# tarepan/ForwardTacotron

Hardware: AMD Instinct MI355X
Metric: mel-frames/sec at batch=64 LJSpeech shapes (ForwardTacotron.generate, B*T_mel per s) (higher is better)
Workload: dtype fp32; 1 GPU; c3: ForwardTacotron generate, batch=64 per GPU, phoneme lengths U{50..200}; global_batch=64, T_phonemes=200, T_mel=1368, parallelism=dp1

## Files before the change

### forwardtacotron_amd/_lib.py

```python
from __future__ import annotations

import ctypes
import os
from pathlib import Path

import torch

from ._srchash import source_hash

_LIB_PATH = Path(os.environ.get('FTMI_LIB', Path(__file__).resolve().parent / 'libftmi.so'))
_lib = None

c_int, c_int64, c_float, c_void_p = ctypes.c_int32, ctypes.c_int64, ctypes.c_float, ctypes.c_void_p
P = c_void_p
ABI_VERSION = 20
MMA_F32, MMA_BF16X6, MMA_F16X3 = 0, 1, 2


class ConvArgs(ctypes.Structure):
    _fields_ = [
        ('x', P), ('x_stride', c_int64), ('B', c_int), ('T', c_int), ('Cin', c_int),
        ('w', P), ('N', c_int), ('k', c_int), ('pad', c_int),
        ('bias', P), ('relu', c_int), ('bn_scale', P), ('bn_shift', P), ('maxpool', c_int),
        ('residual', P), ('res_stride', c_int64),
        ('y', P), ('y_stride', c_int64), ('yt', P), ('T_out', c_int), ('mma', c_int),
        ('split_k', c_int), ('split_ws', P), ('w_split', P), ('status', P), ('x_split', c_int),
    ]


class WaveRNNArgs(ctypes.Structure):
    _fields_ = [(n, P) for n in ('w_hh1', 'w_hh2', 'w_ih2a', 'w_fc1a', 'w_fc2a', 'w_fc3', 'b_fc3',
                                 'b_hh1', 'b_hh2', 'u1', 'u2', 'v1', 'wm', 'cond', 'mel', 'xin',
                                 'samples', 'logits', 'workspace', 'status')] + [
        ('seed', ctypes.c_uint64)] + [(n, c_int) for n in (
            'bias_row', 'item_rows', 'frames_per_item', 'hop', 'fold_stride', 'batched', 'B', 'L',
            'n_classes', 'mol', 'rnn_dims', 'fc_dims', 'feat_dims', 'aux_dims')]


class TacoArgs(ctypes.Structure):
    _fields_ = [(n, P) for n in (
        'enc', 'enc_proj', 'pre_w1t', 'pre_b1', 'pre_w2t', 'pre_b2', 'gru_wih', 'gru_whh', 'gru_bih',
        'gru_bhh', 'lsa_conv', 'lsa_L', 'lsa_Lb', 'lsa_wt', 'lsa_Wb', 'lsa_v', 'rin_w', 'rin_b',
        'l1_wih', 'l1_whh', 'l1_bih', 'l1_bhh', 'l2_wih', 'l2_whh', 'l2_bih', 'l2_bhh', 'mel_w',
        'pre_gi', 'mel_out', 'attn_out', 'steps_out', 'status', 'workspace', 'stamps')] + [
        ('stop_threshold', c_float)] + [(n, c_int) for n in (
            'B', 'T', 'r', 'steps', 'decoder_dims', 'lstm_dims', 'n_mels', 'prenet_dims')]


class NnlsArgs(ctypes.Structure):
    _fields_ = [('mel', P)] + [(n, c_int) for n in ('B', 'F', 'n_mels', 'n_bins', 'denorm')] + [
        ('blocks', P)] + [(n, c_int) for n in ('n_blocks', 'groups', 'm', 'max_frames', 'maxiter', 'dbg_stop')] + [
        (n, P) for n in ('rowvals', 'rowptr', 'rowlo', 'bin_rows', 'bin_w', 'pinv', 'workspace', 'S',
                         'active')]


SIGNATURES = {
    'ftmi_abi_version': (c_int, []),
    'ftmi_build_id': (ctypes.c_char_p, []),
    'ftmi_strerror': (ctypes.c_char_p, [c_int]),
    'ftmi_set_resident_cu_limit': (c_int, [c_int]),
    'ftmi_embedding': (c_int, [P, c_int64, P, c_int64, c_int64, P, P, P]),
    'ftmi_conv1d': (c_int, [ctypes.POINTER(ConvArgs), P]),
    'ftmi_conv_bank': (c_int, [P, c_int64, c_int, c_int, c_int, P, P, c_int, c_int, P, P, P, c_int64,
                               c_int, P, P]),
    'ftmi_conv_bank_split': (c_int, [P, c_int64, c_int, c_int, c_int, P, P, c_int, c_int, P, P, P,
                                     c_int64, c_int, P, c_int, P, c_int, P]),
    'ftmi_conv_bank_halves_ws_floats': (c_int64, [c_int, c_int, c_int, c_int]),
    'ftmi_conv_bank_halves_image_bytes': (c_int64, [c_int, c_int, c_int]),
    'ftmi_conv_bank_halves_image': (c_int, [P, c_int, c_int, c_int, P, P]),
    'ftmi_highway': (c_int, [P, c_int64, c_int64, c_int, P, P, P, P, P, c_int64, c_int, P, P]),
    'ftmi_highway_split': (c_int, [P, c_int64, c_int64, c_int, P, P, P, P, P, c_int64, c_int, P,
                                   c_int, P, P]),
    'ftmi_highway_stack': (c_int, [P, c_int64, c_int64, c_int, c_int, P, c_int, P, P, P, P, P,
                                   c_int, P, c_int64, P, c_int64, P, P]),
    'ftmi_highway_stack_spread_ws_bytes': (c_int64, [c_int64]),
    'ftmi_highway_stack_spread_blocks': (c_int, [c_int64]),
    'ftmi_highway_stack_spread': (c_int, [P, c_int64, c_int64, c_int, c_int, P, c_int, P, P, P, P,
                                          P, c_int, P, c_int64, P, c_int64, P, P, P]),
    'ftmi_split_weights_bytes': (c_int64, [c_int64, c_int64]),
    'ftmi_split_weights': (c_int, [P, c_int64, c_int64, P, P]),
    'ftmi_split_weights_f16_bytes': (c_int64, [c_int64, c_int64]),
    'ftmi_split_rows': (c_int, [P, c_int64, c_int64, c_int, P, c_int64, P, P]),
    'ftmi_split_weights_f16': (c_int, [P, c_int64, c_int64, P, P]),
    'ftmi_split_weights_f16_frag': (c_int, [P, c_int64, c_int64, P, P]),
    'ftmi_panel_proj': (c_int, [P, c_int64, c_int64, c_int, P, c_int, P, P, c_int64, P, P,
                                c_float, P, c_int64, P, P]),
    'ftmi_rnn_workspace_bytes': (c_int64, [c_int, c_int, c_int]),
    'ftmi_rnn_error_offset': (c_int64, [c_int]),
    'ftmi_rnn_blocks': (c_int, [c_int, c_int, c_int, c_int]),
    'ftmi_set_rnn_spin_limit': (ctypes.c_uint32, [ctypes.c_uint32]),
    'ftmi_rnn_bidir': (c_int, [c_int, c_int, c_int, c_int, P, c_int64, c_int, P, P, P, P, P,
                               c_float, P, c_int64, c_int, P, P, P]),
    'ftmi_duration_counts': (c_int, [P, c_int, c_int, c_int, c_float, P, P, P, P]),
    'ftmi_duration_trunc_sum': (c_int, [P, c_int, c_int, P, P]),
    'ftmi_duration_counts_global': (c_int, [P, c_int, c_int, P, c_float, P, P, P, P]),
    'ftmi_lr_index': (c_int, [P, c_int, c_int, c_int, P, P]),
    'ftmi_length_regulate': (c_int, [P, c_int64, c_int, c_int, c_int, P, c_int, P, c_int64, P]),
    'ftmi_series_proj_add': (c_int, [P, c_int64, c_int, c_int, c_int, P, P, P, c_float, P, P, P,
                                     c_float, P]),
    'ftmi_rowdot': (c_int, [P, c_int64, c_int64, c_int, P, P, c_float, P, P]),
    'ftmi_embedding_posenc': (c_int, [P, c_int, c_int, P, c_int64, c_int, P, P, P, P, P]),
    'ftmi_lr_posenc': (c_int, [P, c_int64, c_int, c_int, c_int, P, c_int, P, P, P, c_int64, P]),
    'ftmi_layernorm': (c_int, [P, c_int64, c_int64, c_int, P, P, c_float, P, c_int64, P]),
    'ftmi_attention': (c_int, [P, c_int64, c_int, c_int, c_int, c_int, c_int, c_int, c_int, P,
                               c_float, P, c_int64, c_int, P, P, c_int64, P]),
    'ftmi_panel_proj_qkv': (c_int, [P, c_int64, c_int, c_int, c_int, P, c_int, P, c_int, P,
                                    c_int64, P, c_int64, P, P]),
    'ftmi_attention_kv': (c_int, [P, c_int64, c_int, c_int, c_int, c_int, P, c_float, P, c_int64,
                                  P, P, c_int64, P]),
    'ftmi_attention_workspace_bytes': (c_int64, [c_int, c_int, c_int, c_int]),
    'ftmi_stft': (c_int, [P, c_int64, c_int, c_int64, P, c_int, c_int, P, P, c_int, P, P, P]),
    'ftmi_mel_spectrogram': (c_int, [P, c_int64, c_int, c_int64, P, c_int, c_int, P, P, c_int, P,
                                     P, P, P, c_int, c_int, P, P]),
    'ftmi_griffinlim_stft': (c_int, [P, c_int64, c_int, c_int64, P, c_int, c_int, P, P, c_int, P,
                                     P, P, c_float, c_int, P, P]),
    'ftmi_spec_mul': (c_int, [P, P, c_int64, P, P]),
    'ftmi_unit_phases': (c_int, [P, c_int, c_int, c_int, P, P]),
    'ftmi_istft_workspace_bytes': (c_int64, [c_int, c_int, c_int]),
    'ftmi_istft': (c_int, [P, c_int, c_int, P, c_int, c_int, P, P, P, P, P, c_int64, c_int64, P]),
    'ftmi_griffinlim_iter': (c_int, [P, P, P, P, c_int, c_int, P, c_int, c_int, P, P, P, c_float,
                                     c_int, P]),
    'ftmi_istft_fused': (c_int, [P, c_int, c_int, P, c_int, c_int, P, P, P, P, c_int64, c_int64, P]),
    'ftmi_wr_stretch_conv': (c_int, [P, c_int64, c_int, c_int, c_int, c_int, P, P, c_int64, c_int,
                                     c_int, P]),
    'ftmi_wavernn_workspace_bytes': (c_int64, []),
    'ftmi_wavernn': (c_int, [ctypes.POINTER(WaveRNNArgs), P]),
    'ftmi_set_wavernn_spin_limit': (ctypes.c_uint32, [ctypes.c_uint32]),
    'ftmi_wr_unfold': (c_int, [P, c_int, c_int, c_int, c_int, c_int, c_int, c_int, c_int, c_int, P, P]),
    'ftmi_tacotron_decoder_workspace_bytes': (c_int64, [c_int, c_int]),
    'ftmi_tacotron_decoder': (c_int, [ctypes.POINTER(TacoArgs), P]),
    'ftmi_align_workspace_bytes': (c_int64, [c_int, c_int, c_int]),
    'ftmi_align_dijkstra': (c_int, [P, c_int64, c_int64, c_int, c_int, c_int, P, P, P, P, P, P]),
    'ftmi_align_count': (c_int, [P, c_int64, c_int64, c_int, c_int, c_int, P, P, P, P]),
    'ftmi_attention_score': (c_int, [P, c_int64, c_int64, c_int, c_int, c_int, P, c_int, P, P, P]),
    'ftmi_phoneme_features': (c_int, [P, c_int64, c_int64, c_int, c_int, c_int, P, P, c_int64, c_int,
                                      P, P, c_int64, c_int, P, c_float, P, P, P, P]),
    'ftmi_nonzero_moments': (c_int, [P, c_int64, P, P]),
    'ftmi_normalize_nonzero': (c_int, [P, c_int64, c_float, c_float, P]),
    'ftmi_mel_nnls': (c_int, [P, c_int, c_int, P, c_int, c_int, c_int, c_int, P, P, P, P, P, P,
                              c_float, c_int, P, P]),
    'ftmi_nnls_lbfgsb_workspace_bytes': (c_int64, [c_int, c_int, c_int, c_int, c_int]),
    'ftmi_nnls_lbfgsb_start': (c_int, [ctypes.POINTER(NnlsArgs), P]),
    'ftmi_nnls_lbfgsb_cycles': (c_int, [ctypes.POINTER(NnlsArgs), c_int, P]),
    'ftmi_nnls_lbfgsb_finish': (c_int, [ctypes.POINTER(NnlsArgs), P, P, P, P]),
}


class FtmiError(RuntimeError):
    pass


def lib_path() -> Path:
# ... 32 lines not shown
```

### forwardtacotron_amd/common_layers.py

```python
from __future__ import annotations

import math
from typing import List, Optional

import torch
import torch.nn as nn

from . import ops



def _uniform_(t: torch.Tensor, bound: float) -> None:
    with torch.no_grad():
        t.uniform_(-bound, bound)


class Conv1dParams(nn.Module):

    def __init__(self, cin: int, cout: int, k: int, bias: bool) -> None:
        super().__init__()
        self.in_channels, self.out_channels, self.kernel_size = cin, cout, k
        self.weight = nn.Parameter(torch.empty(cout, cin, k))
        self.bias = nn.Parameter(torch.empty(cout)) if bias else None
        b = 1.0 / math.sqrt(cin * k)
# ... 146 lines not shown

class BiRNN(Packed):

    def __init__(self, fin: int, hidden: int, cell: str) -> None:
        super().__init__()
        self.cell = 0 if cell == 'gru' else 1
        self.input_size, self.hidden = fin, hidden
        self.spread = False
        gh = (3 if self.cell == 0 else 4) * hidden
        b = 1.0 / math.sqrt(hidden)
        for sfx in ('', '_reverse'):
            for name, shape in (('weight_ih_l0', (gh, fin)), ('weight_hh_l0', (gh, hidden)),
                                ('bias_ih_l0', (gh,)), ('bias_hh_l0', (gh,))):
                prm = nn.Parameter(torch.empty(*shape))
                _uniform_(prm, b)
                self.register_parameter(name + sfx, prm)

    def _pack(self):
        w_ih = torch.cat([self.weight_ih_l0, self.weight_ih_l0_reverse], 0).detach().contiguous()
        b_ih = torch.cat([self.bias_ih_l0, self.bias_ih_l0_reverse], 0).detach().contiguous()
        b_hh = torch.cat([self.bias_hh_l0, self.bias_hh_l0_reverse], 0).detach().contiguous()
        w_hh = torch.stack([self.weight_hh_l0, self.weight_hh_l0_reverse], 0).detach().contiguous()
        if self.cell == 1:
            return w_ih, (b_ih + b_hh).contiguous(), None, w_hh, presplit(w_ih)
        return w_ih, b_ih, b_hh, w_hh, presplit(w_ih)

    def forward_cl(self, x: torch.Tensor, T: Optional[int] = None, index=None, lengths=None,
                   pad_value: float = 0.0) -> torch.Tensor:
        return self.recur(self.project(x), T=T, index=index, lengths=lengths,
                          pad_value=pad_value)

    def project(self, x: torch.Tensor) -> torch.Tensor:
        w_ih, b_in, _, _, w3 = self.packed_weights()
        xp, _ = ops.conv1d(x, w_ih, 1, 0, bias=b_in, w_split=w3)
        return xp

    def recur(self, xp: torch.Tensor, T: Optional[int] = None, index=None, lengths=None,
              pad_value: float = 0.0) -> torch.Tensor:
        _, b_in, b_hh, w_hh, _ = self.packed_weights()
        return ops.rnn_bidir(self.cell, xp, self.hidden, w_hh, b_hh, T=T, index=index,
                             xp_zero=b_in if index is not None else None, lengths=lengths,
                             pad_value=pad_value, spread=self.spread)

    def forward(self, x: torch.Tensor):
        return self.forward_cl(x.contiguous()), None


class CBHG(Packed):

    def __init__(self, K: int, in_channels: int, channels: int, proj_channels: List[int],
                 num_highways: int, dropout: float = 0.5) -> None:
        super().__init__()
        self.dropout = dropout
        self.K = K
        self.channels = channels
        self.bank_kernels = list(range(1, K + 1))
        self.conv1d_bank = nn.ModuleList(
            [BatchNormConv(in_channels, channels, k) for k in self.bank_kernels])
        self.conv_project1 = BatchNormConv(K * channels, proj_channels[0], 3)
        self.conv_project2 = BatchNormConv(proj_channels[0], proj_channels[1], 3, relu=False)
        self.pre_highway = LinearParams(proj_channels[-1], channels, bias=False)
        self.highways = nn.ModuleList([HighwayNetwork(channels) for _ in range(num_highways)])
        self.rnn = GRUParamsModule(channels, channels)

    def _pack(self):
        ws = [pack_conv(c.conv.weight) for c in self.conv1d_bank]
        bank_w = torch.cat([w.reshape(-1) for w in ws]).contiguous()
        folds = [c.bnorm.folded() for c in self.conv1d_bank]
        scale = torch.cat([f[0] for f in folds]).contiguous()
        shift = torch.cat([f[1] for f in folds]).contiguous()
        w_pre = self.pre_highway.weight.detach().contiguous()
        bank3 = ops.split_bank_weights(bank_w, self.K, ws[0].size(1), self.channels)
        img = ops.bank_halves_image(bank3, self.K, ws[0].size(1), self.channels)
        return bank_w, scale, shift, w_pre, bank3, presplit(w_pre), img

    def forward_cl(self, x: torch.Tensor) -> torch.Tensor:
        bank_w, scale, shift, w_pre, bank3, pre3, img = self.packed_weights()
        pooled = ops.bank_pools(x, self.K, self.channels, w_split=bank3)
        split = pooled and ops.SPLIT_ROWS
        xin = pooled and ops.SPLIT_BANK_IN
        bank = ops.conv_bank(ops.split_rows(x) if xin else x, bank_w, self.K, self.channels,
                             scale, shift, w_split=bank3, pool=pooled, split_out=split,
                             x_split=xin, w_image=img)
        y = self.conv_project1.forward_cl(bank, maxpool=not pooled, x_split=split)
        del bank
        y = self.conv_project2.forward_cl(y, residual=x)
        xp = self._highway_stack(y)
        if xp is not None:
            return self.rnn.recur(xp)
        h, _ = ops.conv1d(y, w_pre, 1, 0, w_split=pre3)
        h2 = torch.empty_like(h)
        for hw in self.highways:
            hw.forward_cl(h, out=h2)
            h, h2 = h2, h
        return self.rnn.forward_cl(h)

    def _stack_pack(self):
        key = self._pack_key()
        cache = self.__dict__.get('_ftmi_stack')
        if cache is None or cache[0] != key:
            with torch.no_grad():
                w_pre = self.packed_weights()[3]
                hw = [m.packed_weights() for m in self.highways]
                w_ih, b_in = self.rnn.packed_weights()[:2]
                f16 = ops.split_weights_f16
                cache = (key, (f16(w_pre, frag=True), [f16(p[0], frag=True) for p in hw],
                               [p[1] for p in hw], [p[2] for p in hw], f16(w_ih, frag=True),
                               b_in, w_ih.size(0)))
            self.__dict__['_ftmi_stack'] = cache
        return cache[1]

    def spread_blocks(self, M: int) -> int:
        Cp = self.channels
        if not ops.highway_stack_ok(M, Cp, self.channels, len(self.highways), 6 * self.channels,
                                    (self.packed_weights()[5],)):
            return 0
        return ops.hs_spread_blocks(M, 6 * self.channels)

    def _highway_stack(self, y: torch.Tensor) -> Optional[torch.Tensor]:
        M, Cp = y.size(0) * y.size(1), y.size(2)
        n_out = 6 * self.channels
        if not ops.highway_stack_ok(M, Cp, self.channels, len(self.highways), n_out,
                                    (self.packed_weights()[5],)):
            return None
        pre_f, hw_f, b1s, b2s, ih_f, b_in, n_out = self._stack_pack()
        xp, _ = ops.highway_stack(y, pre_f, self.channels, hw_f, b1s, b2s, ih_f, b_in, n_out,
                                  spread=getattr(self, 'allow_spread', True))
        return xp

    def forward(self, x: torch.Tensor) -> torch.Tensor:
        return self.forward_cl(x.transpose(1, 2).contiguous())


class GRUParamsModule(BiRNN):

    def __init__(self, fin: int, hidden: int) -> None:
        super().__init__(fin, hidden, 'gru')


class LSTMParamsModule(BiRNN):

    def __init__(self, fin: int, hidden: int) -> None:
        super().__init__(fin, hidden, 'lstm')
```

### forwardtacotron_amd/forward_tacotron.py

```python
from __future__ import annotations

import os
from pathlib import Path
from typing import Any, Callable, Dict, Union

import numpy as np
import torch
import torch.nn as nn

from . import ops
from .common_layers import (CBHG, BatchNormConv, BiRNN, Conv1dParams, LengthRegulator,
                            LinearParams, Packed, pack_conv)
from .text.symbols import phonemes


def _identity(t: torch.Tensor) -> torch.Tensor:
    return t


def graph_safe(fn: Callable[[torch.Tensor], torch.Tensor]) -> Callable[[torch.Tensor], torch.Tensor]:
    fn._ftmi_graph_safe = True
    return fn


# ... 180 lines not shown
        pitch = batch['pitch'].unsqueeze(1)
        energy = batch['energy'].unsqueeze(1)
        with torch.no_grad():
            dur_hat = self.dur_pred.forward_bt(x)
            pitch_hat = self.pitch_pred.forward_bt(x).unsqueeze(1)
            energy_hat = self.energy_pred.forward_bt(x).unsqueeze(1)
            enc = self._encode(x, pitch, energy)
            dur_c = dur.float().contiguous()
            offsets, totals, _ = ops.duration_counts(dur_c, apply_fill=False)
            if dur_c.data_ptr() != dur.data_ptr():
                dur.copy_(dur_c)
            lens = mel_lens.to(torch.int64)
            T_pack = int(lens.max().item())
            if T_pack > int(totals.max().item()):
                raise RuntimeError('mel_len exceeds the length-regulated sequence length')
            index = ops.lr_index(offsets, T_pack)
            x_mel, x_post = self._decode(enc, index, lengths=lens.to(x.device))
            x_post = self._pad(x_post, mel.size(2))
            x_mel = self._pad(x_mel, mel.size(2))
        return {'mel': x_mel, 'mel_post': x_post,
                'dur': dur_hat, 'pitch': pitch_hat, 'energy': energy_hat}

    def _side_streams(self, device, B: int, T: int = 0):
        cache = self.__dict__.setdefault('_ftmi_streams', {})
        if device not in cache:
            prio = int(os.environ.get('FTMI_PRENET_PRIORITY', '-1'))
            cache[device] = [torch.cuda.Stream(device=device), torch.cuda.Stream(device=device),
                             torch.cuda.Stream(device=device, priority=prio)]
        fits = self.__dict__.setdefault('_ftmi_concurrent', {})
        key = (device, B, T, ops.RNN_MMA, bool(ops._FORCED), os.environ.get('FTMI_HS_SPREAD', '1'))
        if key not in fits:
            preds = (self.dur_pred.rnn, self.pitch_pred.rnn, self.energy_pred.rnn)
            need = sum(ops.rnn_blocks(r.cell, B, r.hidden) for r in preds)
            pre = ops.rnn_blocks(self.prenet.rnn.cell, B, self.prenet.rnn.hidden)
            spread = self.prenet.spread_blocks(B * T)
            cus = ops._num_cus()
            use_spread = spread > 0 and need + max(pre, spread) <= cus
            fits[key] = (0 < need + pre <= cus and pre > 0, use_spread)
        concurrent, use_spread = fits[key]
        self.prenet.allow_spread = use_spread
        if not concurrent:
            main = torch.cuda.current_stream(device)
            return [main, main, main]
        return cache[device]

    def _weights_key(self):
        refs = self.__dict__.get('_ftmi_wrefs')
        if refs is None or any(d.get(n) is not t for d, n, t in refs):
            refs = [(d, n, t) for m in self.modules() for d in (m._parameters, m._buffers)
                    for n, t in d.items() if t is not None]
            self.__dict__['_ftmi_wrefs'] = refs
        return tuple((t.data_ptr(), t._version) for _, _, t in refs)

    def _phoneme_graph(self, x, alpha, pitch_fn, energy_fn):
        cache = self.__dict__.setdefault('_ftmi_graphs', {})
        seen = self.__dict__.setdefault('_ftmi_graph_seen', {})
        split = not (_graphable(pitch_fn) and _graphable(energy_fn))
        key = ((x.device, tuple(x.shape), float(alpha), 'split', ops.MMA, ops.RNN_MMA) if split else
               (x.device, tuple(x.shape), float(alpha), pitch_fn, energy_fn, ops.MMA, ops.RNN_MMA))
        cap_p, cap_e = (None, None) if split else (pitch_fn, energy_fn)
        ent = cache.pop(key, None)
        fresh = False
        if ent is None:
            n = seen.get(key, 0)
            if n < 0:
                return None
            if len(seen) >= 64 * GRAPH_CACHE:
                seen.clear()
            seen[key] = n + 1
            if n == 0:
                return None
            wkey = self._weights_key()
            sx = x.clone()
            try:
                self._phoneme_phase(sx, alpha, cap_p, cap_e, capture=True)
                torch.cuda.synchronize(x.device)
                g = torch.cuda.CUDAGraph()
                with torch.cuda.graph(g):
                    outs = self._phoneme_phase(sx, alpha, cap_p, cap_e, capture=True)
            except Exception:
                torch.cuda.synchronize(x.device)
                seen[key] = -1
                return None
            packs = [m.__dict__.get('_ftmi_pack') for m in self.modules()]
            ent = {'g': g, 'sx': sx, 'outs': outs, 'wkey': wkey, 'packs': packs,
                   'done': torch.cuda.Event()}
            ent['done'].record(torch.cuda.current_stream(x.device))
            fresh = True
            while len(cache) >= GRAPH_CACHE:
                cache.pop(next(iter(cache)))
        cache[key] = ent
        main = torch.cuda.current_stream(x.device)
        main.wait_event(ent['done'])
        ent['sx'].copy_(x)
        ent['g'].replay()
        if not fresh and self._weights_key() != ent['wkey']:
            main.synchronize()
            cache.clear()
            return None
        dur_hat, pitch_hat, energy_hat, enc, offsets, tmax, xp = ent['outs']
        t_host = torch.empty((), dtype=tmax.dtype, pin_memory=True)
        t_host.copy_(tmax, non_blocking=True)
        t_ready = torch.cuda.Event()
        t_ready.record(main)
        dur_hat, pitch_hat, energy_hat = dur_hat.clone(), pitch_hat.clone(), energy_hat.clone()
        if split:
            pitch_hat, energy_hat = pitch_fn(pitch_hat), energy_fn(energy_hat)
            wp, bp, we, be = self._folded_series_weights()
            ops.series_proj_add(xp, pitch_hat, wp, bp, self.pitch_strength, energy_hat, we,
                                be, self.energy_strength)
        t_ready.synchronize()
        return (dur_hat, pitch_hat, energy_hat, enc, offsets, int(t_host), xp), ent

    def _phoneme_phase(self, x, alpha, pitch_fn, energy_fn, batch=None, capture=False):
        main = torch.cuda.current_stream(x.device)
        s_pitch, s_energy, s_prenet = self._side_streams(x.device, x.size(0), x.size(1))
        for s in (s_pitch, s_energy, s_prenet):
            s.wait_stream(main)
        with torch.cuda.stream(s_prenet):
            enc = self.prenet.forward_cl(ops.embedding(x, self.embedding.weight.detach()))
            xp = self.lstm.project(enc)
        dur_hat = self.dur_pred.forward_bt(x, alpha=alpha)
        t_host = t_ready = None
        tmax = None
        if batch is None and capture:
            offsets, totals, _ = ops.duration_counts(dur_hat, apply_fill=True)
            tmax = totals.max()
        elif batch is None:
            offsets, totals, _ = ops.duration_counts(dur_hat, apply_fill=True)
            t_host = torch.empty((), dtype=totals.dtype, pin_memory=True)
            t_host.copy_(totals.max(), non_blocking=True)
            t_ready = torch.cuda.Event()
            t_ready.record(main)
        with torch.cuda.stream(s_pitch):
            pitch_hat = self.pitch_pred.forward_bt(x).unsqueeze(1)
            if pitch_fn is not None:
                pitch_hat = pitch_fn(pitch_hat)
        with torch.cuda.stream(s_energy):
            energy_hat = self.energy_pred.forward_bt(x).unsqueeze(1)
            if energy_fn is not None:
                energy_hat = energy_fn(energy_hat)
        if pitch_fn is not None and energy_fn is not None:
            with torch.cuda.stream(s_prenet):
                for s, t in ((s_pitch, pitch_hat), (s_energy, energy_hat)):
                    s_prenet.wait_stream(s)
                    if not capture:
                        t.record_stream(s_prenet)
                wp, bp, we, be = self._folded_series_weights()
                ops.series_proj_add(xp, pitch_hat, wp, bp, self.pitch_strength, energy_hat, we,
                                    be, self.energy_strength)
        if batch is not None:
            offsets, totals = batch.duration_counts(dur_hat)
            T_mel = batch.t_mel(totals)
        index = None
        if not capture:
            if t_ready is not None:
                t_ready.synchronize()
                T_mel = int(t_host)
            index = ops.lr_index(offsets, T_mel)
        for s, ts in ((s_pitch, (pitch_hat,)), (s_energy, (energy_hat,)),
                      (s_prenet, (enc, xp))):
            main.wait_stream(s)
            if not capture:
                for t in ts:
                    t.record_stream(main)
        if capture:
            return dur_hat, pitch_hat, energy_hat, enc, offsets, tmax, xp
        return dur_hat, pitch_hat, energy_hat, enc, (offsets, index), T_mel, xp

    def generate(self,
                 x: torch.Tensor,
                 alpha=1.0,
                 pitch_function: Callable[[torch.Tensor], torch.Tensor] = _identity,
                 energy_function: Callable[[torch.Tensor], torch.Tensor] = _identity,
                 batch=None) -> Dict[str, torch.Tensor]:
        if self.training:
            self.eval()
        self._check_device(x)

        graph = GRAPH and batch is None and x.numel() <= GRAPH_MAX_TOKENS

        def run():
            with torch.no_grad():
                phase = ent = None
                if graph and not ops.forced_exact():
                    r = self._phoneme_graph(x, alpha, pitch_function, energy_function)
                    if r is not None:
                        phase, ent = r
                if phase is None:
                    phase = self._phoneme_phase(x, alpha, pitch_function, energy_function, batch)
                dur_hat, pitch_hat, energy_hat, enc, offsets, T_mel, xp = phase
                out = self._generate_mel(x, dur_hat, pitch_hat, energy_hat, enc=enc,
                                         lr=(offsets, T_mel), xp=xp)
                if ent is not None:
                    ent['done'].record(torch.cuda.current_stream(x.device))
                return out
        return ops.run_checked(run, x.device, reduce=None if batch is None else batch.status)

    def __prepare_scriptable__(self):
        from .jit import ScriptedForwardTacotron
        return ScriptedForwardTacotron(self)

    def generate_jit(self, x: torch.Tensor, alpha: float = 1.0, beta: float = 1.0) -> Dict[str, torch.Tensor]:
        self._check_device(x)

        def run():
            with torch.no_grad():
                dur_hat, pitch_hat, energy_hat, enc, offsets, T_mel, xp = self._phoneme_phase(
                    x, alpha, lambda p: p * beta, lambda e: e)
                return self._generate_mel(x, dur_hat, pitch_hat, energy_hat, enc=enc,
                                          lr=(offsets, T_mel), xp=xp)
        return ops.run_checked(run, x.device)

    def get_step(self) -> int:
        return self.step.data.item()

    def _generate_mel(self, x, dur_hat, pitch_hat, energy_hat, enc=None, lr=None, xp=None):
        if enc is None:
            enc = self.prenet.forward_cl(ops.embedding(x, self.embedding.weight.detach()))
        if xp is None:
            wp, bp, we, be = self._series_proj_weights()
            ops.series_proj_add(enc, pitch_hat, wp, bp, self.pitch_strength, energy_hat, we, be,
                                self.energy_strength)
        index = None
        if lr is None:
            offsets, totals, _ = ops.duration_counts(dur_hat, apply_fill=False)
            T_mel = int(totals.max().item())
        else:
            offsets, T_mel = lr
            if isinstance(offsets, tuple):
                offsets, index = offsets
        if index is None:
            index = ops.lr_index(offsets, T_mel)
        mel, mel_post = self._decode(enc, index, xp=xp)
        return {'mel': mel, 'mel_post': mel_post, 'dur': dur_hat,
                'pitch': pitch_hat, 'energy': energy_hat}

    def _pad(self, x: torch.Tensor, max_len: int) -> torch.Tensor:
        x = x[:, :, :max_len]
        if x.size(2) < max_len:
            pad = torch.full((x.size(0), x.size(1), max_len - x.size(2)), self.padding_value,
                             device=x.device, dtype=x.dtype)
            x = torch.cat([x, pad], 2)
        return x

    @classmethod
    def from_config(cls, config: Dict[str, Any]) -> 'ForwardTacotron':
        model_config = config['forward_tacotron']['model']
        model_config['num_chars'] = len(phonemes)
        model_config['n_mels'] = config['dsp']['num_mels']
        return ForwardTacotron(**model_config)

    @classmethod
    def from_checkpoint(cls, path: Union[Path, str]) -> 'ForwardTacotron':
        checkpoint = torch.load(path, map_location=torch.device('cpu'), weights_only=True)
        model = ForwardTacotron.from_config(checkpoint['config'])
        model.load_state_dict(checkpoint['model'])
        return model
```

### forwardtacotron_amd/ops.py

```python
from __future__ import annotations

import contextlib
import ctypes
import os
from typing import Optional, Tuple

import numpy as np
import torch

from . import _lib
from ._lib import ConvArgs
from .probe import launch

_f32 = torch.float32

MMA = int(os.environ.get('FTMI_MMA', '2'))
RNN_MMA = int(os.environ.get('FTMI_RNN_MMA', '2'))

STATUS_F16_RANGE, STATUS_WHH_RANGE, STATUS_RNN_TIMEOUT = 1, 2, 4
_STATUS = {}
_FORCED = []


def status_word(device) -> torch.Tensor:
# ... 284 lines not shown
                      Cout: int) -> Optional[torch.Tensor]:
    if (w_split is None or w_split.dtype != torch.uint8 or not w_split.is_cuda
            or os.environ.get('FTMI_BANK_IMAGE', '1') == '0'):
        return None
    lib = _lib.load()
    n = int(lib.ftmi_conv_bank_halves_image_bytes(Cin, K, Cout))
    if n <= 0:
        return None
    img = torch.empty(n, device=w_split.device, dtype=torch.uint8)
    launch('ftmi_conv_bank_halves_image', f'bank_halves_image[K={K},Cin={Cin},Cout={Cout}]', 0,
           2.0 * n, w_split.data_ptr(), Cin, K, Cout, img.data_ptr(), _stream())
    return img


def conv_bank(x: torch.Tensor, w: torch.Tensor, K: int, Cout: int, scale: torch.Tensor,
              shift: torch.Tensor, mma: Optional[int] = None,
              w_split: Optional[torch.Tensor] = None, pool: bool = False,
              split_out: bool = False, x_split: bool = False,
              w_image: Optional[torch.Tensor] = None) -> torch.Tensor:
    if split_out and not pool:
        raise ValueError('split_out needs pool')
    _dev(x, w, scale, shift, w_split)
    B, T, Cin, xs = _rows(x)
    y = torch.empty(B, T, K * Cout, device=x.device, dtype=_f32)
    M = B * T
    flops = 2.0 * M * Cout * Cin * K * (K + 1) / 2
    mma, wsp = _gemm_mma(mma, w_split)
    sk, part, last = 0, None, 0
    if not pool and not x_split and _bank_halves(mma, B, T, Cin, K, Cout):
        n = int(_lib.load().ftmi_conv_bank_halves_ws_floats(B, T, K, Cout)) - BANK_COUNTERS
        sk, part, last = 2, _bank_workspace(n, x.device), BANK_HALVES
        if w_image is not None:
            _dev(w_image)
            wsp, last = w_image.data_ptr(), BANK_HALVES | BANK_IMAGE
    elif not pool and _skinny(mma, T, T, Cin, K, M) and _skinny_split(Cin) > 1:
        sk = _skinny_split(Cin)
        part = torch.empty(sk * M * K * Cout, device=x.device, dtype=_f32)
    launch('ftmi_conv_bank_split', f'conv_bank[M={M},K={K},Cin={Cin},mma={mma}'
           f'{",pool" if pool else ""}{",split" if split_out else ""}{",xsplit" if x_split else ""}'
           ']',
           flops, 4.0 * (M * Cin + Cout * Cin * K * (K + 1) / 2 + M * K * Cout),
           x.data_ptr(), xs, B, T, Cin, w.data_ptr(), wsp, K, Cout,
           scale.data_ptr(), shift.data_ptr(), y.data_ptr(), y.stride(-2), mma,
           status_word(x.device).data_ptr(), sk, _ptr(part),
           int(pool) | (2 * int(split_out)) | (4 * int(x_split)) | last, _stream())
    return y


BANK_COUNTERS = 4096
BANK_HALVES, BANK_IMAGE = 16, 32


def _bank_halves(mma: int, B: int, T: int, Cin: int, K: int, Cout: int) -> bool:
    return (os.environ.get('FTMI_BANK_HALVES', '1') != '0' and mma == 2 and 0 < B * T <= 128
            and Cin % 64 == 0 and Cin <= 256 and K % 2 == 0 and Cout % 16 == 0
            and (K // 2) * (Cout // 16) % 8 == 0 and (K // 2) * (Cout // 16) <= 512 and K <= 16)
_BANK_WS = {}


def _bank_workspace(n_part: int, device) -> torch.Tensor:
    stream = torch.cuda.current_stream(device)
    key = (torch.device(device), stream.cuda_stream)
    t = _BANK_WS.get(key)
    if t is None or t.numel() < BANK_COUNTERS + n_part:
        if t is not None:
            _BANK_OLD.append(t)
        t = _BANK_WS[key] = torch.zeros(BANK_COUNTERS + n_part, device=device, dtype=_f32)
    return t


_BANK_OLD = []


def split_rows(x: torch.Tensor) -> torch.Tensor:
    _dev(x)
    B, T, C, xs = _rows(x)
    y = torch.empty(B, T, C, device=x.device, dtype=_f32)
    launch('ftmi_split_rows', f'split_rows[M={B * T},C={C}]', 0.0, 8.0 * B * T * C,
           x.data_ptr(), xs, B * T, C, y.data_ptr(), y.stride(1),
           status_word(x.device).data_ptr(), _stream())
    return y


def highway(x: torch.Tensor, w12: torch.Tensor, b1: torch.Tensor, b2: torch.Tensor,
            out: Optional[torch.Tensor] = None, mma: Optional[int] = None,
            w_split: Optional[torch.Tensor] = None) -> torch.Tensor:
    _dev(x, w12, b1, b2, out, w_split)
    B, T, C, xs = _rows(x)
    y = out if out is not None else torch.empty(B, T, C, device=x.device, dtype=_f32)
    M = B * T
    mma, wsp = _gemm_mma(mma, w_split)
    sk, part = 0, None
    if (mma == 2 and wsp is not None and os.environ.get('FTMI_GEMM_SKINNY', '1') != '0'
            and C % 16 == 0 and 0 < M <= SKINNY_MMAX_NARROW):
        sk = _skinny_split(C)
        part = torch.empty(sk * M * 2 * C, device=x.device, dtype=_f32)
    launch('ftmi_highway_split', f'highway[M={M},C={C},mma={mma}]', 2.0 * M * 2 * C * C,
           4.0 * (2 * M * C + 2 * C * C),
           x.data_ptr(), xs, M, C, w12.data_ptr(), wsp, b1.data_ptr(),
           b2.data_ptr(), y.data_ptr(), y.stride(1), mma, status_word(x.device).data_ptr(),
           sk, _ptr(part), _stream())
    return y


HS_C, HS_NPASS, HS_MAXL = 256, 512, 8
HS_MIN_ROWS = int(os.environ.get('FTMI_HS_MIN', 64))


def highway_stack_ok(M: int, Cp: int, C: int, L: int, n_out: int, splits) -> bool:
    if os.environ.get('FTMI_HS', '1') == '0' or (_FORCED and _FORCED[-1][0] != 2):
        return False
    if not _FORCED and MMA != 2:
        return False
    return (C == HS_C and 0 < Cp <= C and Cp % 4 == 0 and L <= HS_MAXL
            and n_out % HS_NPASS == 0 and M >= max(HS_MIN_ROWS, 1)
            and all(w is not None and w.dtype == torch.uint8 for w in splits))


def highway_stack(x: torch.Tensor, pre_split: torch.Tensor, C: int, hw_splits, b1s, b2s,
                  out_split: Optional[torch.Tensor], b_out: Optional[torch.Tensor], n_out: int,
                  want_h: bool = False, spread: bool = True):
    _dev(x, pre_split, out_split, b_out, *hw_splits, *b1s, *b2s)
    B, T, Cp, xs = _rows(x)
    M = B * T
    L = len(hw_splits)
    y = torch.empty(B, T, n_out, device=x.device, dtype=_f32) if out_split is not None else None
    h = torch.empty(B, T, C, device=x.device, dtype=_f32) if want_h else None
    arr = ctypes.c_void_p * max(L, 1)
    w_arr = arr(*[w.data_ptr() for w in hw_splits])
    b1_arr = arr(*[b.data_ptr() for b in b1s])
    b2_arr = arr(*[b.data_ptr() for b in b2s])
    flops = 2.0 * M * C * (Cp + L * 2 * C + n_out)
    nbytes = 4.0 * M * (Cp + n_out + (C if want_h else 0))
    args = (x.data_ptr(), xs, M, Cp, C, pre_split.data_ptr(), L, ctypes.addressof(w_arr),
            ctypes.addressof(b1_arr), ctypes.addressof(b2_arr), _ptr(out_split), _ptr(b_out),
            n_out if out_split is not None else 0, _ptr(y), y.stride(1) if y is not None else 0,
            _ptr(h), h.stride(1) if h is not None else 0, status_word(x.device).data_ptr())
    if spread and hs_spread_blocks(M, n_out if out_split is not None else 0) > 0:
        ws = _spread_workspace(int(_lib.load().ftmi_highway_stack_spread_ws_bytes(M)), x.device)
        launch('ftmi_highway_stack_spread', f'highway_stack_spread[M={M},Cp={Cp},L={L},N={n_out}]',
               flops, nbytes, *args, ws.data_ptr(), _stream())
    else:
        launch('ftmi_highway_stack', f'highway_stack[M={M},Cp={Cp},L={L},N={n_out}]', flops,
               nbytes, *args, _stream())
    return y, h


def hs_spread_blocks(M: int, n_out: int = 0) -> int:
    if os.environ.get('FTMI_HS_SPREAD', '1') == '0' or n_out > 1536:
        return 0
    n = int(_lib.load().ftmi_highway_stack_spread_blocks(M))
    return n if 0 < n <= _num_cus() else 0


_SPREAD_WS = {}


def _spread_workspace(nbytes: int, device) -> torch.Tensor:
    stream = torch.cuda.current_stream(device)
    key = (torch.device(device), stream.cuda_stream)
    t = _SPREAD_WS.get(key)
    if t is None or t.numel() < nbytes:
        if t is not None:
            _BANK_OLD.append(t)
        t = _SPREAD_WS[key] = torch.zeros(max(nbytes, 16), device=device, dtype=torch.uint8)
    return t
# ... 487 lines not shown
```

### include/ftmi.h

```cpp
#ifndef FTMI_H
#define FTMI_H

#include <stdint.h>

#ifdef __cplusplus
extern "C" {
#endif

typedef void *ftmi_stream_t;

enum {
  FTMI_OK = 0,
  FTMI_E_ARG = 1001,
  FTMI_E_SHAPE = 1002,
  FTMI_E_UNSUPPORTED = 1003,
  FTMI_E_ALIGN = 1004
};

enum { FTMI_MMA_F32 = 0, FTMI_MMA_BF16X6 = 1, FTMI_MMA_F16X3 = 2 };

enum { FTMI_STATUS_F16_RANGE = 1, FTMI_STATUS_WHH_RANGE = 2, FTMI_STATUS_RNN_TIMEOUT = 4 };

enum { FTMI_BANK_POOL = 1,
       FTMI_BANK_Y_SPLIT = 2,
       FTMI_BANK_X_SPLIT = 4,
       FTMI_BANK_HALVES = 16,
       FTMI_BANK_IMAGE = 32    };
enum { FTMI_BANK_COUNTERS = 4096 };

int ftmi_abi_version(void);
const char *ftmi_build_id(void);
const char *ftmi_strerror(int code);
int32_t ftmi_set_resident_cu_limit(int32_t cus);

int ftmi_embedding(const int64_t *ids, int64_t n, const float *table, int64_t num_rows,
                   int64_t dim, float *out, int32_t *err, ftmi_stream_t stream);

typedef struct ftmi_conv_args {
  const float *x;
  int64_t x_stride;
  int32_t B, T, Cin;
  const float *w;
  int32_t N, k, pad;
  const float *bias;
  int32_t relu;
  const float *bn_scale;
  const float *bn_shift;
  int32_t maxpool;
  const float *residual;
  int64_t res_stride;
  float *y;
  int64_t y_stride;
  float *yt;
  int32_t T_out;
  int32_t mma;
  int32_t split_k;
  float *split_ws;
  const void *w_split;
  uint32_t *status;
  int32_t x_split;
} ftmi_conv_args;


int64_t ftmi_split_weights_bytes(int64_t N, int64_t K);
int ftmi_split_weights(const float *w, int64_t N, int64_t K, void *out, ftmi_stream_t stream);

int64_t ftmi_split_weights_f16_bytes(int64_t N, int64_t K);
int ftmi_split_weights_f16(const float *w, int64_t N, int64_t K, void *out,
                           ftmi_stream_t stream);

int ftmi_conv1d(const ftmi_conv_args *args, ftmi_stream_t stream);

int ftmi_conv_bank(const float *x, int64_t x_stride, int32_t B, int32_t T, int32_t Cin,
                   const float *w, const void *w_split, int32_t K, int32_t Cout,
                   const float *bn_scale,
                   const float *bn_shift, float *y, int64_t y_stride, int32_t mma,
                   uint32_t *status, ftmi_stream_t stream);

int64_t ftmi_conv_bank_halves_ws_floats(int32_t B, int32_t T, int32_t K, int32_t Cout);
int64_t ftmi_conv_bank_halves_image_bytes(int32_t Cin, int32_t K, int32_t Cout);
int ftmi_conv_bank_halves_image(const void *w_split, int32_t Cin, int32_t K, int32_t Cout,
                                void *image, ftmi_stream_t stream);
int ftmi_conv_bank_split(const float *x, int64_t x_stride, int32_t B, int32_t T, int32_t Cin,
                         const float *w, const void *w_split, int32_t K, int32_t Cout,
                         const float *bn_scale, const float *bn_shift, float *y,
                         int64_t y_stride, int32_t mma, uint32_t *status, int32_t split_k,
                         float *split_ws, int32_t pool_out, ftmi_stream_t stream);

int ftmi_highway(const float *x, int64_t x_stride, int64_t M, int32_t C, const float *w12,
                 const void *w12_split, const float *b1, const float *b2, float *y,
                 int64_t y_stride, int32_t mma, uint32_t *status, ftmi_stream_t stream);

int ftmi_highway_split(const float *x, int64_t x_stride, int64_t M, int32_t C,
                       const float *w12, const void *w12_split, const float *b1,
                       const float *b2, float *y, int64_t y_stride, int32_t mma,
                       uint32_t *status, int32_t split_k, float *split_ws,
                       ftmi_stream_t stream);

int ftmi_split_weights_f16_frag(const float *w, int64_t N, int64_t K, void *out,
                                ftmi_stream_t stream);

int ftmi_split_rows(const float *x, int64_t x_stride, int64_t rows, int32_t C, float *y,
                    int64_t y_stride, uint32_t *status, ftmi_stream_t stream);

int ftmi_highway_stack(const float *x, int64_t x_stride, int64_t M, int32_t Cp, int32_t C,
                       const void *w_pre_split, int32_t L, const void *const *w_hw_split,
                       const float *const *b1, const float *const *b2,
                       const void *w_out_split, const float *b_out, int32_t n_out, float *y,
                       int64_t y_stride, float *h, int64_t h_stride, uint32_t *status,
                       ftmi_stream_t stream);

int64_t ftmi_highway_stack_spread_ws_bytes(int64_t M);
int32_t ftmi_highway_stack_spread_blocks(int64_t M);
int ftmi_highway_stack_spread(const float *x, int64_t x_stride, int64_t M, int32_t Cp,
                              int32_t C, const void *w_pre_split, int32_t L,
                              const void *const *w_hw_split, const float *const *b1,
                              const float *const *b2, const void *w_out_split,
                              const float *b_out, int32_t n_out, float *y, int64_t y_stride,
                              float *h, int64_t h_stride, uint32_t *status, void *ws,
                              ftmi_stream_t stream);

enum { FTMI_RNN_SPREAD = 0x100 };
int64_t ftmi_rnn_workspace_bytes(int32_t B, int32_t H, int32_t cell);
int64_t ftmi_rnn_error_offset(int32_t B);
int32_t ftmi_rnn_blocks(int32_t cell, int32_t B, int32_t H, int32_t mma);
uint32_t ftmi_set_rnn_spin_limit(uint32_t limit);
int ftmi_rnn_bidir(int32_t cell, int32_t B, int32_t T, int32_t H, const float *xp,
                   int64_t xp_stride, int32_t T_src, const int32_t *index,
                   const float *xp_zero, const float *w_hh, const float *b_hh,
                   const int32_t *lengths, float pad_value, float *y, int64_t y_stride,
                   int32_t mma, uint32_t *status, void *sync, ftmi_stream_t stream);

int ftmi_duration_counts(float *dur, int32_t B, int32_t T, int32_t apply_fill,
                         float fill_value, int32_t *offsets, int32_t *totals,
                         int32_t *fill_flag, ftmi_stream_t stream);

int ftmi_duration_trunc_sum(const float *dur, int32_t B, int32_t T, int64_t *out,
                            ftmi_stream_t stream);
int ftmi_duration_counts_global(float *dur, int32_t B, int32_t T, const int64_t *global_sum,
                                float fill_value, int32_t *offsets, int32_t *totals,
                                int32_t *fill_flag, ftmi_stream_t stream);

int ftmi_lr_index(const int32_t *offsets, int32_t B, int32_t T, int32_t T_mel,
                  int32_t *index, ftmi_stream_t stream);

int ftmi_length_regulate(const float *x, int64_t x_stride, int32_t B, int32_t T, int32_t C,
                         const int32_t *index, int32_t T_mel, float *y, int64_t y_stride,
                         ftmi_stream_t stream);

int ftmi_series_proj_add(float *x, int64_t x_stride, int32_t B, int32_t T, int32_t C,
                         const float *pitch, const float *wp, const float *bp,
                         float pitch_strength, const float *energy, const float *we,
                         const float *be, float energy_strength, ftmi_stream_t stream);

int ftmi_rowdot(const float *x, int64_t x_stride, int64_t M, int32_t C, const float *w,
                const float *bias, float alpha, float *out, ftmi_stream_t stream);


int ftmi_stft(const float *y, int64_t y_stride, int32_t B, int64_t L, const int32_t *lengths,
              int32_t n_fft, int32_t hop, const double *window, const void *twiddle, int32_t F,
              const int32_t *frames, void *X, ftmi_stream_t stream);

int ftmi_mel_spectrogram(const float *y, int64_t y_stride, int32_t B, int64_t L,
                         const int32_t *lengths, int32_t n_fft, int32_t hop, const double *window,
                         const void *twiddle, int32_t F, const int32_t *frames, const float *basis,
                         const int32_t *mel_lo, const int32_t *mel_hi, int32_t n_mels,
                         int32_t log_norm, float *mel, ftmi_stream_t stream);

int ftmi_griffinlim_stft(const float *y, int64_t y_stride, int32_t B, int64_t L,
                         const int32_t *lengths, int32_t n_fft, int32_t hop, const double *window,
                         const void *twiddle, int32_t F, const int32_t *frames, const float *S,
// ... 162 lines not shown
```

Baseline: 10.99 million mel-frames/s.

## Fold embedding into CBHG conv bank via precomputed per-token tap table

Because the prenet CBHG conv bank's input is an embedding lookup, each bank convolution output becomes a sum of precomputed rows, one per (token id, tap), from a table built as embedding times conv weight. A new kernel gathers and sums these rows, then applies ReLU, batchnorm, maxpool and the optional f16 split output, replacing the conv-bank GEMM. The table is cached per weight version and registered with the graph pack list. It trades matmul compute for table memory and gather bandwidth, which grows with vocab times taps times Cout.

```diff
diff --git a/forwardtacotron_amd/_lib.py b/forwardtacotron_amd/_lib.py
--- a/forwardtacotron_amd/_lib.py
+++ b/forwardtacotron_amd/_lib.py
@@ -68,6 +68,8 @@
     'ftmi_conv_bank_halves_ws_floats': (c_int64, [c_int, c_int, c_int, c_int]),
     'ftmi_conv_bank_halves_image_bytes': (c_int64, [c_int, c_int, c_int]),
     'ftmi_conv_bank_halves_image': (c_int, [P, c_int, c_int, c_int, P, P]),
+    'ftmi_embed_bank': (c_int, [P, c_int, c_int, P, c_int, c_int, c_int, c_int, P, P, P, c_int64,
+                                c_int, P, P]),
     'ftmi_highway': (c_int, [P, c_int64, c_int64, c_int, P, P, P, P, P, c_int64, c_int, P, P]),
     'ftmi_highway_split': (c_int, [P, c_int64, c_int64, c_int, P, P, P, P, P, c_int64, c_int, P,
                                    c_int, P, P]),
diff --git a/forwardtacotron_amd/common_layers.py b/forwardtacotron_amd/common_layers.py
--- a/forwardtacotron_amd/common_layers.py
+++ b/forwardtacotron_amd/common_layers.py
@@ -252,6 +252,35 @@
         bank = ops.conv_bank(ops.split_rows(x) if xin else x, bank_w, self.K, self.channels,
                              scale, shift, w_split=bank3, pool=pooled, split_out=split,
                              x_split=xin, w_image=img)
+        return self._after_bank(bank, x, pooled, split)
+
+    def embed_bank_table(self, embedding_weight: torch.Tensor) -> torch.Tensor:
+        key = (self._pack_key(), embedding_weight.data_ptr(), embedding_weight._version,
+               embedding_weight.device)
+        cache = self.__dict__.get('_ftmi_embed_table')
+        if cache is None or cache[0] != key:
+            with torch.no_grad():
+                cache = (key, ops.embed_bank_table(
+                    embedding_weight, [c.conv.weight for c in self.conv1d_bank]))
+            self.__dict__['_ftmi_embed_table'] = cache
+        return cache[1]
+
+    def forward_ids(self, x_ids: torch.Tensor, embedding_weight: torch.Tensor) -> torch.Tensor:
+        w = embedding_weight.detach()
+        h = ops.embedding(x_ids, w)
+        if (x_ids.numel() < ops.EMBED_BANK_MIN_ROWS
+                or w.size(1) != self.conv1d_bank[0].conv.in_channels
+                or not ops.embed_bank_ok(w.size(0), 1, self.K, self.channels)):
+            return self.forward_cl(h)
+        _, scale, shift, _, bank3 = self.packed_weights()[:5]
+        split = ops.SPLIT_ROWS and ops.bank_pools(h, self.K, self.channels, w_split=bank3)
+        bank = ops.embed_bank(x_ids, self.embed_bank_table(w), 1, self.K, self.channels, scale,
+                              shift, pool=True, split_out=split)
+        return self._after_bank(bank, h, True, split)
+
+    def _after_bank(self, bank: torch.Tensor, x: torch.Tensor, pooled: bool,
+                    split: bool) -> torch.Tensor:
+        bank_w, scale, shift, w_pre, bank3, pre3, img = self.packed_weights()
         y = self.conv_project1.forward_cl(bank, maxpool=not pooled, x_split=split)
         del bank
         y = self.conv_project2.forward_cl(y, residual=x)
diff --git a/forwardtacotron_amd/csrc/embed_bank.hip b/forwardtacotron_amd/csrc/embed_bank.hip
--- /dev/null
+++ b/forwardtacotron_amd/csrc/embed_bank.hip
@@ -0,0 +1,223 @@
+#include "common.h"
+
+namespace {
+
+typedef _Float16 f16x4 __attribute__((ext_vector_type(4)));
+typedef decltype(__builtin_amdgcn_make_buffer_rsrc((void *)nullptr, (short)0, 0, 0)) EbRsrc;
+
+constexpr int EB_ROWS = 16;
+constexpr int EB_WAVES = 4;
+constexpr int EB_KMAX = 16;
+constexpr int EB_PANEL = 256;
+constexpr float EB_TAIL = 2048.f;
+
+struct EbParams {
+  const int64_t *ids;
+  int T, M;
+  const float *tab;
+  int S, taps, Cout;
+  int kmin, kmax, slices;
+  const float *scale, *shift;
+  float *y;
+  int64_t y_stride;
+  int pool, split;
+  unsigned *status;
+};
+
+__device__ __forceinline__ f32x4 eb_max4(f32x4 a, f32x4 b) {
+  return (f32x4){fmaxf(a.x, b.x), fmaxf(a.y, b.y), fmaxf(a.z, b.z), fmaxf(a.w, b.w)};
+}
+
+__device__ __forceinline__ int eb_tap_base(int k, int kmin) {
+  return (k * (k - 1) - kmin * (kmin - 1)) / 2;
+}
+
+template <int K>
+struct EbGroup {
+  f32x4 v[K];
+  bool ok[K];
+  f32x4 sc, sh, prev;
+  unsigned tap0;
+
+  __device__ __forceinline__ void init(const EbParams &p, int k, unsigned col) {
+    const int g = k - p.kmin;
+    sc = *(const f32x4 *)(p.scale + (int64_t)g * p.Cout + col);
+    sh = *(const f32x4 *)(p.shift + (int64_t)g * p.Cout + col);
+    prev = (f32x4){0.f, 0.f, 0.f, 0.f};
+    tap0 = (unsigned)eb_tap_base(k, p.kmin);
+  }
+  __device__ __forceinline__ void load(const EbParams &p, EbRsrc rs, unsigned voff, int idv,
+                                       int wlo, int r, int t) {
+#pragma unroll
+    for (int j = 0; j < K; ++j) {
+      const int d = j - K / 2;
+      const int id = __builtin_amdgcn_readlane(idv, r + d - wlo);
+      ok[j] = (unsigned)(t + d) < (unsigned)p.T && id >= 0;
+      const unsigned row = (unsigned)(ok[j] ? id : 0) * (unsigned)p.taps + tap0 + j;
+      v[j] = __builtin_bit_cast(
+          f32x4, __builtin_amdgcn_raw_buffer_load_b128(rs, voff, row * (unsigned)p.Cout * 4u, 0));
+    }
+  }
+  __device__ __forceinline__ f32x4 finish(bool pool_prev) {
+    f32x4 acc = {0.f, 0.f, 0.f, 0.f};
+#pragma unroll
+    for (int j = 0; j < K; ++j) acc += ok[j] ? v[j] : (f32x4){0.f, 0.f, 0.f, 0.f};
+    f32x4 o = eb_max4(acc, (f32x4){0.f, 0.f, 0.f, 0.f});
+    o = o * sc + sh;
+    const f32x4 out = pool_prev ? eb_max4(prev, o) : o;
+    prev = o;
+    return out;
+  }
+  __device__ __forceinline__ bool nan() const {
+    return prev.x != prev.x || prev.y != prev.y || prev.z != prev.z || prev.w != prev.w;
+  }
+};
+template <>
+struct EbGroup<0> {
+  __device__ __forceinline__ void init(const EbParams &, int, unsigned) {}
+  __device__ __forceinline__ void load(const EbParams &, EbRsrc, unsigned, int, int, int, int) {}
+  __device__ __forceinline__ f32x4 finish(bool) { return (f32x4){0.f, 0.f, 0.f, 0.f}; }
+  __device__ __forceinline__ bool nan() const { return false; }
+};
+
+__device__ __forceinline__ bool eb_store(const EbParams &p, int r, int ycol, f32x4 o) {
+  if (p.split) {
+    const f16x4 h = __builtin_convertvector(o, f16x4);
+    const f16x4 t =
+        __builtin_convertvector((o - __builtin_convertvector(h, f32x4)) * EB_TAIL, f16x4);
+    _Float16 *yr = (_Float16 *)(p.y + (int64_t)r * p.y_stride) + ycol;
+    *(f16x4 *)yr = h;
+    *(f16x4 *)(yr + (int64_t)(p.kmax - p.kmin + 1) * p.Cout) = t;
+    return !(fabsf(o.x) <= 65504.f) || !(fabsf(o.y) <= 65504.f) || !(fabsf(o.z) <= 65504.f) ||
+           !(fabsf(o.w) <= 65504.f);
+  }
+  *(f32x4 *)(p.y + (int64_t)r * p.y_stride + ycol) = o;
+  return false;
+}
+
+template <int KA, int KB>
+__device__ __forceinline__ void eb_run(const EbParams &p, int idv, int wlo, int r0, int r1,
+                                       int ka, int kb, int col) {
+  EbGroup<KA> A;
+  EbGroup<KB> Bg;
+  A.init(p, ka, col);
+  Bg.init(p, kb, col);
+  const int ycolA = (ka - p.kmin) * p.Cout + col, ycolB = (kb - p.kmin) * p.Cout + col;
+  const EbRsrc rs = __builtin_amdgcn_make_buffer_rsrc(
+      (void *)p.tab, (short)0, (int)((unsigned)p.S * p.taps * p.Cout * 4u), 0x00020000);
+  const unsigned voff = (unsigned)col * 4u;
+  int t = r0 % p.T;
+  int r = r0;
+  if (p.pool && t > 0) {
+    --r;
+    --t;
+  }
+  bool bad = false;
+  for (; r < r1; ++r) {
+    A.load(p, rs, voff, idv, wlo, r, t);
+    Bg.load(p, rs, voff, idv, wlo, r, t);
+    const bool pool_prev = p.pool && t > 0;
+    const f32x4 oa = A.finish(pool_prev);
+    const f32x4 ob = Bg.finish(pool_prev);
+    if (p.split) bad |= A.nan() || Bg.nan();
+    if (r >= r0) {
+      bad |= eb_store(p, r, ycolA, oa);
+      if (KB > 0) bad |= eb_store(p, r, ycolB, ob);
+    }
+    if (++t == p.T) t = 0;
+  }
+  if (bad && p.status) atomicOr(p.status, 1u);
+}
+
+#define EB_CASES(F)                                                                        \
+  F(1) F(2) F(3) F(4) F(5) F(6) F(7) F(8) F(9) F(10) F(11) F(12) F(13) F(14) F(15) F(16)
+
+__device__ __forceinline__ void eb_single(const EbParams &p, int idv, int wlo, int r0, int r1,
+                                          int k, int col) {
+  switch (k) {
+#define EB_ONE(K_) \
+  case K_: eb_run<K_, 0>(p, idv, wlo, r0, r1, k, k, col); break;
+    EB_CASES(EB_ONE)
+#undef EB_ONE
+    default: break;
+  }
+}
+
+__global__ __launch_bounds__(EB_WAVES * 64, 4) void embed_bank_kernel(const EbParams p) {
+  const int lane = threadIdx.x & 63;
+  const int wave = __builtin_amdgcn_readfirstlane(threadIdx.x >> 6);
+  const int slice = blockIdx.x % p.slices;
+  const int tile = blockIdx.x / p.slices;
+  const int r0 = (tile * EB_WAVES + wave) * EB_ROWS;
+  if (r0 >= p.M) return;
+  const int r1 = min(r0 + EB_ROWS, p.M);
+  const int col = blockIdx.y * EB_PANEL + lane * 4;
+
+  const int wlo = r0 - 1 - EB_KMAX / 2;
+  int idv = -1;
+  {
+    const int m = wlo + lane;
+    if (m >= 0 && m < p.M) {
+      const int64_t id = p.ids[m];
+      if (id >= 0 && id < p.S) idv = (int)id;
+    }
+  }
+  const int ka = p.kmin + slice, kb = p.kmax - slice;
+  if (kb > ka && ka + kb == EB_KMAX + 1) {
+    switch (ka) {
+#define EB_PAIR(K_) \
+  case K_: eb_run<K_, EB_KMAX + 1 - K_>(p, idv, wlo, r0, r1, ka, kb, col); break;
+      EB_PAIR(1) EB_PAIR(2) EB_PAIR(3) EB_PAIR(4) EB_PAIR(5) EB_PAIR(6) EB_PAIR(7) EB_PAIR(8)
+#undef EB_PAIR
+      default: break;
+    }
+    return;
+  }
+  eb_single(p, idv, wlo, r0, r1, ka, col);
+  if (kb > ka) eb_single(p, idv, wlo, r0, r1, kb, col);
+}
+
+}
+
+extern "C" int ftmi_embed_bank(const int64_t *ids, int32_t B, int32_t T, const float *table,
+                               int32_t num_rows, int32_t kmin, int32_t kmax, int32_t Cout,
+                               const float *bn_scale, const float *bn_shift, float *y,
+                               int64_t y_stride, int32_t flags, uint32_t *status,
+                               ftmi_stream_t stream) {
+  if (!ids || !table || !bn_scale || !bn_shift || !y || B <= 0 || T <= 0 || num_rows <= 0 ||
+      Cout <= 0 || kmin < 1 || kmax < kmin)
+    return FTMI_E_ARG;
+  if (flags & ~(FTMI_BANK_POOL | FTMI_BANK_Y_SPLIT)) return FTMI_E_ARG;
+  if (kmax > EB_KMAX || Cout % EB_PANEL) return FTMI_E_UNSUPPORTED;
+  const int G = kmax - kmin + 1;
+  const int64_t taps = (kmax * (kmax + 1) - kmin * (kmin - 1)) / 2;
+  if ((int64_t)num_rows * taps * Cout * 4 >= ((int64_t)1 << 31)) return FTMI_E_UNSUPPORTED;
+  if ((int64_t)B * T > INT32_MAX - 64 || y_stride < (int64_t)G * Cout) return FTMI_E_SHAPE;
+  if (!ftmi_aligned16(table) || !ftmi_aligned16(bn_scale) || !ftmi_aligned16(bn_shift) ||
+      !ftmi_aligned16(y) || (y_stride & 3))
+    return FTMI_E_ALIGN;
+  EbParams p = {};
+  p.ids = ids;
+  p.T = T;
+  p.M = B * T;
+  p.tab = table;
+  p.S = num_rows;
+  p.taps = (int)taps;
+  p.Cout = Cout;
+  p.kmin = kmin;
+  p.kmax = kmax;
+  p.slices = (G + 1) / 2;
+  p.scale = bn_scale;
+  p.shift = bn_shift;
+  p.y = y;
+  p.y_stride = y_stride;
+  p.pool = (flags & FTMI_BANK_POOL) != 0;
+  p.split = (flags & FTMI_BANK_Y_SPLIT) != 0;
+  p.status = status;
+  const int64_t tiles = ((int64_t)p.M + EB_WAVES * EB_ROWS - 1) / (EB_WAVES * EB_ROWS);
+  if (tiles * p.slices > INT32_MAX) return FTMI_E_SHAPE;
+  hipLaunchKernelGGL(embed_bank_kernel, dim3((unsigned)(tiles * p.slices), Cout / EB_PANEL),
+                     dim3(EB_WAVES * 64), 0, ftmi_hs(stream), p);
+  FTMI_CHECK_LAUNCH();
+  return FTMI_OK;
+}
diff --git a/forwardtacotron_amd/forward_tacotron.py b/forwardtacotron_amd/forward_tacotron.py
--- a/forwardtacotron_amd/forward_tacotron.py
+++ b/forwardtacotron_amd/forward_tacotron.py
@@ -286,7 +286,8 @@
                 torch.cuda.synchronize(x.device)
                 seen[key] = -1
                 return None
-            packs = [m.__dict__.get('_ftmi_pack') for m in self.modules()]
+            packs = [m.__dict__.get(k) for m in self.modules()
+                     for k in ('_ftmi_pack', '_ftmi_stack', '_ftmi_embed_table')]
             ent = {'g': g, 'sx': sx, 'outs': outs, 'wkey': wkey, 'packs': packs,
                    'done': torch.cuda.Event()}
             ent['done'].record(torch.cuda.current_stream(x.device))
@@ -322,7 +323,7 @@
         for s in (s_pitch, s_energy, s_prenet):
             s.wait_stream(main)
         with torch.cuda.stream(s_prenet):
-            enc = self.prenet.forward_cl(ops.embedding(x, self.embedding.weight.detach()))
+            enc = self.prenet.forward_ids(x, self.embedding.weight)
             xp = self.lstm.project(enc)
         dur_hat = self.dur_pred.forward_bt(x, alpha=alpha)
         t_host = t_ready = None
@@ -421,7 +422,7 @@
 
     def _generate_mel(self, x, dur_hat, pitch_hat, energy_hat, enc=None, lr=None, xp=None):
         if enc is None:
-            enc = self.prenet.forward_cl(ops.embedding(x, self.embedding.weight.detach()))
+            enc = self.prenet.forward_ids(x, self.embedding.weight)
         if xp is None:
             wp, bp, we, be = self._series_proj_weights()
             ops.series_proj_add(enc, pitch_hat, wp, bp, self.pitch_strength, energy_hat, we, be,
diff --git a/forwardtacotron_amd/ops.py b/forwardtacotron_amd/ops.py
--- a/forwardtacotron_amd/ops.py
+++ b/forwardtacotron_amd/ops.py
@@ -390,6 +390,53 @@
     return y
 
 
+EMBED_BANK_MIN_ROWS = 256
+EMBED_BANK_TILE = (16, 64)
+EMBED_BANK_KMAX, EMBED_BANK_PANEL = 16, 256
+
+
+def embed_bank_taps(kmin: int, kmax: int) -> int:
+    return (kmax * (kmax + 1) - kmin * (kmin - 1)) // 2
+
+
+def embed_bank_table(emb: torch.Tensor, conv_weights) -> torch.Tensor:
+    _dev(emb, *conv_weights)
+    e = emb.detach().double()
+    parts = [torch.einsum('ncj,sc->sjn', w.detach().double(), e) for w in conv_weights]
+    return torch.cat(parts, 1).float().contiguous()
+
+
+def embed_bank_ok(num_rows: int, kmin: int, kmax: int, Cout: int) -> bool:
+    return (1 <= kmin <= kmax <= EMBED_BANK_KMAX and Cout > 0 and Cout % EMBED_BANK_PANEL == 0
+            and num_rows * embed_bank_taps(kmin, kmax) * Cout * 4 < 1 << 31)
+
+
+def embed_bank(ids: torch.Tensor, table: torch.Tensor, kmin: int, kmax: int, Cout: int,
+               scale: torch.Tensor, shift: torch.Tensor, pool: bool = False,
+               split_out: bool = False) -> torch.Tensor:
+    _dev(ids, table, scale, shift)
+    ids = ids.contiguous()
+    if ids.dtype != torch.int64:
+        ids = ids.long()
+    B, T = ids.shape
+    G, taps = kmax - kmin + 1, embed_bank_taps(kmin, kmax)
+    if table.dim() != 3 or table.size(1) != taps or table.size(2) != Cout or table.dtype != _f32 \
+            or not table.is_contiguous():
+        raise ValueError(f'embed_bank: table {tuple(table.shape)} is not contiguous fp32 '
+                         f'[S][{taps}][{Cout}]')
+    if scale.numel() != G * Cout or shift.numel() != G * Cout:
+        raise ValueError('embed_bank: scale / shift must hold G*Cout values')
+    y = torch.empty(B, T, G * Cout, device=table.device, dtype=_f32)
+    M = B * T
+    launch('ftmi_embed_bank', f'embed_bank[M={M},{f"K={kmax}" if kmin == 1 else f"k={kmin}-{kmax}"},'
+           f'Cout={Cout}{",pool" if pool else ""}{",split" if split_out else ""}]',
+           1.0 * M * taps * Cout, 4.0 * M * taps * Cout + 8.0 * M + 4.0 * M * G * Cout,
+           ids.data_ptr(), B, T, table.data_ptr(), table.size(0), kmin, kmax, Cout,
+           scale.data_ptr(), shift.data_ptr(), y.data_ptr(), y.stride(-2),
+           int(pool) | (2 * int(split_out)), status_word(table.device).data_ptr(), _stream())
+    return y
+
+
 def highway(x: torch.Tensor, w12: torch.Tensor, b1: torch.Tensor, b2: torch.Tensor,
             out: Optional[torch.Tensor] = None, mma: Optional[int] = None,
             w_split: Optional[torch.Tensor] = None) -> torch.Tensor:
diff --git a/include/ftmi.h b/include/ftmi.h
--- a/include/ftmi.h
+++ b/include/ftmi.h
@@ -87,6 +87,11 @@
                          int64_t y_stride, int32_t mma, uint32_t *status, int32_t split_k,
                          float *split_ws, int32_t pool_out, ftmi_stream_t stream);
 
+int ftmi_embed_bank(const int64_t *ids, int32_t B, int32_t T, const float *table,
+                    int32_t num_rows, int32_t kmin, int32_t kmax, int32_t Cout,
+                    const float *bn_scale, const float *bn_shift, float *y, int64_t y_stride,
+                    int32_t flags, uint32_t *status, ftmi_stream_t stream);
+
 int ftmi_highway(const float *x, int64_t x_stride, int64_t M, int32_t C, const float *w12,
                  const void *w12_split, const float *b1, const float *b2, float *y,
                  int64_t y_stride, int32_t mma, uint32_t *status, ftmi_stream_t stream);
```

After: 11.35 million mel-frames/s, median of 6. +3.3%, better.
